# wangxuanx/Face-Diffusion-Model

Hardware: AMD Instinct MI355X
Metric: animated frames/sec (1000-step DDPM, VOCASET FDM) at 1/2/4/8 MI355X (higher is better)
Workload: dtype bf16; 1 GPU; cfg2: vocaset FDM, 4 clips/GPU x 200 latent frames, 1000-step DDPM, random-init weights, synthetic audio-encoder features, Philox noise; global_batch=4, latent_frames=200, diffusion_steps=1000, parallelism=clip-shard x1

## Files before the change

### face-diffusion-model_amd/csrc/fdm_hip.hip

```cpp
#include <hip/hip_runtime.h>

#include <algorithm>
#include <cstdarg>
#include <cstdio>
#include <cstring>
#include <functional>
#include <string>
#include <vector>

#include "../../include/fdm_hip.h"
#include "elementwise.hpp"
#include "window.hpp"
#include "kernels.hpp"

namespace fdm {
thread_local std::string g_err;
int fail(int code, const char* fmt, ...) {
  char buf[512];
  va_list ap;
  va_start(ap, fmt);
  vsnprintf(buf, sizeof(buf), fmt, ap);
  va_end(ap);
  g_err = buf;
  return code;
// ... 176 lines not shown
}

int fdm_op_layernorm(const fdm_ln_args* a, void* stream) {
  if (!a || !a->x || !a->gamma || !a->beta) return fail(FDM_ERR_ARG, "layernorm: null operand");
  if (a->d != 256 && a->d != 512 && a->d != 768 && a->d != 1024) return fail(FDM_ERR_SHAPE, "layernorm: d=%d unsupported (256, 512, 768, 1024)", a->d);
  if (a->M <= 0) return fail(FDM_ERR_SHAPE, "layernorm: M must be positive");
  if (!a->y_f32 && !a->y_t) return fail(FDM_ERR_ARG, "layernorm: no output");
  if (a->dtype < FDM_F32 || a->dtype > FDM_F16) return fail(FDM_ERR_ARG, "layernorm: bad dtype %d", a->dtype);
  if (a->y_t && a->dtype == FDM_F16X3 && (a->y_t_lo_off <= 0 || a->y_t_lo_off % 4)) return fail(FDM_ERR_ARG, "layernorm: split y_t needs y_t_lo_off");
  if (a->add_mat_group < 0 || a->add_mat_wrap < 0 ||
      (a->add_mat_group > 0 && (a->add_mat_L <= 0 || a->add_mat_group % a->add_mat_L || (a->add_mat_wrap > 0 && a->add_mat_wrap % a->add_mat_group))))
    return fail(FDM_ERR_SHAPE, "layernorm: shared add_mat needs add_mat_L | add_mat_group | add_mat_wrap (got %d, %d, %d)", a->add_mat_L, a->add_mat_group, a->add_mat_wrap);
  if (a->x_planes < 0 || a->x_planes > 4 || (a->x_planes > 1 && (a->x_plane_stride < (long long)a->M * a->d || a->x_plane_stride % 4)))
    return fail(FDM_ERR_ARG, "layernorm: x_planes %d (0..4) needs x_plane_stride >= M * d, a multiple of 4", a->x_planes);
  fdm_ln_args c = *a;
  return submit([c](hipStream_t s) {
    switch (c.dtype) {
      case FDM_BF16: return fdm::ln_launch_t<fdm::bf16>(c, s);
      case FDM_F16X3: return fdm::ln_launch_t<fdm::f16x3_t>(c, s);
      case FDM_F16: return fdm::ln_launch_t<fdm::f16>(c, s);
      default: return fdm::ln_launch_t<float>(c, s);
    }
  }, stream, "layernorm");
}

int fdm_op_sched_step(const fdm_sched_args* a, void* stream) {
  if (!a || !a->x0 || !a->x_out) return fail(FDM_ERR_ARG, "sched: null operand");
  if (a->n <= 0 || a->n % 4) return fail(FDM_ERR_SHAPE, "sched: n=%lld must be a positive multiple of 4", a->n);
  if (a->mode == 0 && (!a->x || !a->c1 || !a->c2 || !a->sigma)) return fail(FDM_ERR_ARG, "sched: DDPM tables missing");
  if (a->mode == 1 && (!a->x || !a->sra || !a->srm1 || !a->sqrt_an || !a->c_n)) return fail(FDM_ERR_ARG, "sched: DDIM tables missing");
  if (a->mode < 0 || a->mode > 2) return fail(FDM_ERR_ARG, "sched: bad mode %d", a->mode);
  if (a->mode == 0 && !a->noise && (a->n_per_clip <= 0 || a->n_per_clip % 4)) return fail(FDM_ERR_SHAPE, "sched: n_per_clip must be a positive multiple of 4");
  if (a->x_out_t && (a->out_dtype < FDM_F32 || a->out_dtype > FDM_F16)) return fail(FDM_ERR_ARG, "sched: bad out_dtype %d", a->out_dtype);
  if (a->x_out_t && a->out_dtype == FDM_F16X3 && (a->x_out_t_lo_off <= 0 || a->x_out_t_lo_off % 4)) return fail(FDM_ERR_ARG, "sched: split x_out_t needs x_out_t_lo_off");
  fdm_sched_args c = *a;
  return submit([c](hipStream_t s) { return fdm::sched_launch(c, s); }, stream, "sched");
}

}

int fdm::window_sched_op(const fdm_sched_args& a, const fdm::WinArgs& w, void* stream) {
  if (!a.x || !w.off || !w.ent || !w.xw || (!w.init && (!a.x0 || !a.x_out))) return fail(FDM_ERR_ARG, "window_sched: null operand");
  if (a.n <= 0 || a.n % 4 || w.d % 4 || w.L_total < 1 || w.W < 1 || w.n_win < 1 || a.n % ((long long)w.L_total * w.d))
    return fail(FDM_ERR_SHAPE, "window_sched: n=%lld is not a whole number of long clips of %d x %d", a.n, w.L_total, w.d);
  fdm_sched_args c = a;
  fdm::WinArgs ww = w;
// ... 279 lines not shown
```

### face-diffusion-model_amd/csrc/gemm_bf16.hip

```cpp
#include "gemm.hpp"
#include "kernels.hpp"
namespace fdm { hipError_t gemm_launch_bf16(const fdm_gemm_args& a, hipStream_t s) { return gemm_dispatch<bf16>(a, s); } }
namespace fdm {
int gemm_heuristic_tile_of(const fdm_gemm_args& a) {
  if (a.ksplit > 1) return gemm_ksplit_heuristic_tile(a);
  if (a.sched_fuse) {
    const bool pp = a.dtype != FDM_F16X3 && gemm_tile_override() == 0 && !a.ln_stat_in && a.N % 128 == 0 && gemm_sched_fuse_heuristic_pp(a, a.dtype == FDM_F32 ? 4 : 2);
    return pp ? FDM_TILE_256x128_PP : FDM_TILE_64x64;
  }
  const int want = gemm_tile_override();
  if (want > 0) return want;
  return gemm_heuristic_tile(a, a.dtype == FDM_F32 ? 4 : 2, a.dtype == FDM_F16X3);
}
}
```

### face-diffusion-model_amd/csrc/gemm_f16.hip

```cpp
#include "gemm.hpp"
#include "kernels.hpp"
namespace fdm { hipError_t gemm_launch_f16(const fdm_gemm_args& a, hipStream_t s) { return gemm_dispatch<f16>(a, s); } }
```

### face-diffusion-model_amd/csrc/kernels.hpp

```cpp
#pragma once
#include <hip/hip_runtime.h>
#include "../../include/fdm_hip.h"

namespace fdm {
int fail(int code, const char* fmt, ...);
hipError_t gemm_launch_f32(const fdm_gemm_args& a, hipStream_t s);
hipError_t gemm_launch_bf16(const fdm_gemm_args& a, hipStream_t s);
hipError_t gemm_launch_f16x3(const fdm_gemm_args& a, hipStream_t s);
hipError_t gemm_launch_f16(const fdm_gemm_args& a, hipStream_t s);
int gemm_heuristic_tile_of(const fdm_gemm_args& a);
hipError_t attn_launch_f32(const fdm_attn_args& a, hipStream_t s);
hipError_t attn_launch_bf16(const fdm_attn_args& a, hipStream_t s);
hipError_t attn_launch_f16x3(const fdm_attn_args& a, hipStream_t s);
hipError_t attn_launch_f16(const fdm_attn_args& a, hipStream_t s);
hipError_t pack_kv_launch_f32(const void* K, long long ldk, const void* V, long long ldv, void* Kp, void* Vp, int B, int H, int L, int Lpad, int hd, hipStream_t s);
hipError_t pack_kv_launch_bf16(const void* K, long long ldk, const void* V, long long ldv, void* Kp, void* Vp, int B, int H, int L, int Lpad, int hd, hipStream_t s);

struct WinEnt { int w; int start; float wt; int pad; };
struct WinArgs {
  const int* off; const WinEnt* ent;
  float* xw;
  int L_total;
  int n_win;
  int W;
  int d;
  int init;
};
int window_sched_op(const fdm_sched_args& p, const WinArgs& w, void* stream);

inline hipError_t gemm_launch(const fdm_gemm_args& a, hipStream_t s) {
  switch (a.dtype) {
    case FDM_BF16: return gemm_launch_bf16(a, s);
// ... 10 lines not shown
```

### face-diffusion-model_amd/csrc/plan.hip

```cpp
#include <hip/hip_runtime.h>

#include <algorithm>
#include <cmath>
#include <cstdint>
#include <cstdio>
#include <cstdlib>
#include <cstring>
#include <fstream>
#include <map>
#include <set>
#include <string>
#include <vector>

#include <unistd.h>

#include "../../include/fdm_hip.h"
#include "common.hpp"
#include "kernels.hpp"

namespace {
using fdm::fail;

#define HIPCK(x) do { hipError_t e_ = (x); if (e_ != hipSuccess) return fail(FDM_ERR_HIP, "%s: %s", #x, hipGetErrorString(e_)); } while (0)
#define FCK(x) do { int r_ = (x); if (r_ != FDM_OK) return r_; } while (0)
// ... 214 lines not shown
  void *q = nullptr, *kp = nullptr, *vp = nullptr;
  long long q_lo = 0, kv_lo = 0;
  size_t kv_bytes = 0;
  float *AF = nullptr, *t1 = nullptr, *sty = nullptr, *em = nullptr, *emu = nullptr, *zeros = nullptr, *E0 = nullptr;
  std::vector<float*> C1;
  int* step = nullptr;
  unsigned long long* seedbuf = nullptr;
  int* tseq = nullptr; int tseq_cap = 0;
  std::map<int, std::pair<int, float*>> ddim;
  std::map<int, std::vector<int>> ddim_t;
  std::map<std::string, fdm_prog*> progs;
  std::vector<std::string> prog_order;
  std::vector<std::string> pinned;
  std::map<std::string, int> tiles;
  std::map<std::string, std::map<std::string, int>> tile_cache;
  std::map<std::string, long long> steps_seen;
  std::map<std::string, std::vector<fdm_gemm_args>>* tune_rec = nullptr;
  int tune_enabled = 1;
  int tune_failed = 0;
  std::set<std::string> tune_failed_shapes;
  int want_fuse_ln3 = 0;
  int ksplit_out = 1, ksplit_ffn2 = 1;
  int x1_planes = 0;
  int lockstep = 0;
  int tune_lazy = 0;
  long long last_graph_launches = 0, launches_per_step = 0;
  int win_n = 0, win_len = 0, win_total = 0, win_overlap = 0, win_B = 0;
  float* xlong = nullptr; size_t xlong_cap = 0;
  int* win_off = nullptr; size_t win_off_cap = 0;
  fdm::WinEnt* win_ent = nullptr; size_t win_ent_cap = 0;
  float* win_stage = nullptr; size_t win_stage_cap = 0;
};

namespace {

size_t esize(int dtype) { return dtype == FDM_F32 ? 4 : 2; }
bool is_split(int dtype) { return dtype == FDM_F16X3; }

int dalloc(fdm_plan* P, void** out, size_t bytes, bool ws, bool zero = true) {
  void* p = nullptr;
  HIPCK(hipMalloc(&p, bytes ? bytes : 16));
  if (zero) HIPCK(hipMemset(p, 0, bytes ? bytes : 16));
  (ws ? P->ws_allocs : (P->in_commit ? P->commit_allocs : P->allocs)).push_back(p);
  *out = p;
  return FDM_OK;
}
// ... 37 lines not shown
  *out = w->p;
  return FDM_OK;
}

fdm_gemm_args gemm_f32(const float* A, const float* W, int M, int N, int K) {
  fdm_gemm_args a;
  memset(&a, 0, sizeof(a));
  a.A = A; a.lda = K; a.W = W; a.ldw = K; a.M = M; a.N = N; a.K = K; a.batch = 1; a.dtype = FDM_F32;
  a.ldr = N; a.ldo_f32 = N; a.ldo_t = N; a.ln_eps = 1e-5f;
  return a;
}
fdm_gemm_args gemm_op(const fdm_plan* P, const Mat& A, const Mat& W, int M, int N, int K) {
  fdm_gemm_args a = gemm_f32((const float*)A.p, (const float*)W.p, M, N, K);
  a.dtype = P->dtype; a.a_lo_off = A.lo; a.w_lo_off = W.lo;
  return a;
}
void set_out_t(fdm_gemm_args& a, const Mat& o) { a.out_t = o.p; a.out_t_lo_off = o.lo; }

int to_operand(fdm_plan* P, const float* src, long long n, Mat* out, void* stream) {
  if (P->dtype == FDM_F32) { out->p = (void*)src; out->lo = 0; return FDM_OK; }
  out->lo = is_split(P->dtype) ? n : 0;
  FCK(dalloc(P, &out->p, (size_t)n * 2 * (is_split(P->dtype) ? 2 : 1), false, false));
  return fdm_op_cast(src, out->p, n, P->dtype, stream);
}

int plan_gemm(fdm_plan* P, const char* label, fdm_gemm_args a, void* stream) {
  if (P->tune_rec) (*P->tune_rec)[label].push_back(a);
  auto it = P->tiles.find(label);
  a.tile = (it == P->tiles.end() ? 0 : it->second) | (P->lockstep ? FDM_TILE_LOCKSTEP : 0);
  return fdm_op_gemm(&a, stream);
}

std::string lname(int l, const char* suffix) {
  char b[96];
  snprintf(b, sizeof(b), "transformer_decoder.layers.%d.%s", l, suffix);
  return b;
}

int commit_impl(fdm_plan* P, void* stream) {
  const fdm_model_desc& m = P->m;
  const int d = m.d;
  hipStream_t s = (hipStream_t)stream;
  FCK(drop_programs(P, stream));
  const float* p = nullptr;
  FCK(need(P, "audio_extract.0.weight", (long long)d * m.audio_in, &p));
  FCK(need(P, "audio_extract.0.bias", d, &p));
// ... 225 lines not shown
    at.scale = 1.0f / std::sqrt((float)P->hd); at.causal = 1; at.slopes = P->slopes; at.period = m.period;
    if (split) { at.q_lo_off = P->q_lo; at.kv_lo_off = P->kv_lo; at.o_lo_off = P->ctx.lo; }
    FCK(fdm_op_attention(&at, stream));
    FCK(need(P, lname(l, "self_attn.out_proj.bias"), d, &b));
    g = gemm_op(P, P->ctx, P->wt[lname(l, "self_attn.out_proj.weight")], R, d, d);
    g.bias = b; g.out_f32 = P->x1;
    if (!f) {
      g.resid = P->h;
      if (P->ksplit_out > 1) { g.ksplit = P->ksplit_out; g.ksplit_stride = (long long)R * d; }
      FCK(plan_gemm(P, "out", g, stream));
    } else {
      g.resid = P->x2; g.ln_stat_in = P->stats; g.ln_nparts = np; g.ln_dim = d; g.ln_eps = eps; g.rln_gamma = f->gamma; g.rln_beta = f->beta;
      FCK(plan_gemm(P, "out_ln", g, stream));
    }
    fdm_ln_args ln;
    memset(&ln, 0, sizeof(ln));
    ln.x = P->x1; ln.M = R; ln.d = d; ln.add_mat = P->C1[l]; ln.add_tab = P->TT[l]; ln.tab_step = tcur; ln.eps = eps;
    if (P->S > 1) { ln.add_mat_L = L; ln.add_mat_group = P->S * L; ln.add_mat_wrap = M; }
    if (!f && P->ksplit_out > 1) { ln.x_planes = P->ksplit_out; ln.x_plane_stride = (long long)R * d; }
    FCK(need(P, lname(l, "norm1.weight"), d, &ln.gamma)); FCK(need(P, lname(l, "norm1.bias"), d, &ln.beta));
    FCK(need(P, lname(l, "norm2.weight"), d, &ln.gamma2)); FCK(need(P, lname(l, "norm2.bias"), d, &ln.beta2));
    ln.y_f32 = P->h2; ln.dtype = P->dtype;
    if (both) { ln.y_t = P->h2t.p; ln.y_t_lo_off = P->h2t.lo; }
    FCK(fdm_op_layernorm(&ln, stream));
    FCK(need(P, lname(l, "linear1.bias"), m.ffn, &b));
    g = gemm_op(P, P->h2t, P->wt[lname(l, "linear1.weight")], R, m.ffn, d);
    g.bias = b; g.act = FDM_ACT_RELU; set_out_t(g, P->u);
    FCK(plan_gemm(P, "ffn1", g, stream));
    FCK(need(P, lname(l, "linear2.bias"), d, &b));
    g = gemm_op(P, P->u, P->wt[lname(l, "linear2.weight")], R, d, m.ffn);
    g.bias = b; g.resid = P->h2;
    if (fuse) {
      g.out_f32 = P->x2; set_out_t(g, P->x2t); g.stat_out = P->stats;
      FCK(plan_gemm(P, "ffn2_stat", g, stream));
    } else {
      g.out_f32 = P->x1;
      if (P->ksplit_ffn2 > 1) { g.ksplit = P->ksplit_ffn2; g.ksplit_stride = (long long)R * d; }
      FCK(plan_gemm(P, "ffn2", g, stream));
      memset(&ln, 0, sizeof(ln));
      ln.x = P->x1; ln.M = R; ln.d = d; ln.eps = eps; ln.y_f32 = P->h; ln.dtype = P->dtype;
      if (P->ksplit_ffn2 > 1) { ln.x_planes = P->ksplit_ffn2; ln.x_plane_stride = (long long)R * d; }
      FCK(need(P, lname(l, "norm3.weight"), d, &ln.gamma)); FCK(need(P, lname(l, "norm3.bias"), d, &ln.beta));
      if (both) { ln.y_t = P->ht.p; ln.y_t_lo_off = P->ht.lo; }
      FCK(fdm_op_layernorm(&ln, stream));
    }
  }
  fdm_gemm_args g;
  if (fuse) {
    const Fold& f = P->fold[-1];
    g = gemm_op(P, P->x2t, f.w, R, d, d);
    g.bias = f.bias; g.ln_stat_in = P->stats; g.ln_nparts = np; g.ln_dim = d; g.ln_eps = eps; g.ln_colsum = f.colsum;
// ... 3 lines not shown
    g.bias = b;
  }
  if (sched) {
    g.resid = P->x; g.out_f32 = P->x;
    if (both) set_out_t(g, P->xt);
    g.sched_fuse = 1; g.sched = *sched;
  } else {
    g.out_f32 = P->x0;
  }
  return plan_gemm(P, fuse ? "dec_ln" : "dec", g, stream);
}

struct ProgSpec {
  int kind;
  const float* noise = nullptr; float cfg_scale = 0.f;
  const float* san = nullptr; const float* cn = nullptr;
  int reps = 1;
};

std::string tiles_sig(const fdm_plan* P) {
  std::string s;
  for (auto& kv : P->tiles)
    if (kv.second) s += kv.first + "=" + std::to_string(kv.second) + ",";
  s += "ks" + std::to_string(P->ksplit_out) + std::to_string(P->ksplit_ffn2) + (P->lockstep ? "L" : "");
  return s;
}

fdm::WinArgs win_args(const fdm_plan* P, int init) {
  fdm::WinArgs w;
  w.off = P->win_off; w.ent = P->win_ent; w.xw = P->x;
  w.L_total = P->win_total; w.n_win = P->win_n; w.W = P->win_len; w.d = P->m.d; w.init = init;
  return w;
}

int get_program(fdm_plan* P, const ProgSpec& sp, void* stream, fdm_prog** out) {
  char key[512];
  snprintf(key, sizeof(key), "%s#%s|%d|%p|%a|%p|%d", shape_key(P).c_str(), tiles_sig(P).c_str(), sp.kind, (const void*)sp.noise, (double)sp.cfg_scale,
           (const void*)sp.san, sp.reps);
  if (P->win_n) {
    const size_t kl = strlen(key);
    snprintf(key + kl, sizeof(key) - kl, "|win%d,%d,%d,%d,%d", P->win_B, P->win_total, P->win_n, P->win_len, P->win_overlap);
  }
  auto it = P->progs.find(key);
  if (it != P->progs.end()) {
    auto pos = std::find(P->prog_order.begin(), P->prog_order.end(), std::string(key));
    if (pos != P->prog_order.end()) { P->prog_order.erase(pos); P->prog_order.push_back(key); }
    P->pinned.push_back(key);
// ... 324 lines not shown
  if (any) {
    float t_h = 0.f, t_t = 0.f;
    FCK(chain_time({}, &t_h));
    FCK(chain_time(tuned, &t_t));
    for (auto& kv : runner_up) {
      std::map<std::string, int> trial = tuned;
      trial[kv.first] = kv.second;
      float t_a = 0.f;
      FCK(chain_time(trial, &t_a));
      if (t_a < 0.997f * t_t) { tuned = trial; t_t = t_a; }
    }
    if (t_t < 0.99f * t_h) {
      float t_h2 = 0.f;
      FCK(chain_time({}, &t_h2));
      t_h = std::min(t_h, t_h2);
    }
    if (t_t < 0.99f * t_h) keep = tuned;
    if (getenv("FDM_TUNE_VERBOSE")) {
      std::string desc;
      for (auto& kv : tuned) desc += kv.first + "=" + std::to_string(kv.second) + ",";
      fprintf(stderr, "[fdm tune] rows=%d candidates: %s chain %.3f -> %.3f ms: %s\n", P->R, desc.c_str(), t_h / 4, t_t / 4, keep.empty() ? "rejected" : "kept");
    }
  }
  P->tiles = keep;
  apply_tile_override(P->tiles);
  P->tile_cache[key] = P->tiles;
  return FDM_OK;
}

}

extern "C" {

int fdm_plan_create(const fdm_model_desc* desc, int B, int L, int cfg, int dtype, fdm_plan** out) {
  if (!desc || !out) return fail(FDM_ERR_ARG, "plan_create: null argument");
  if (dtype < FDM_F32 || dtype > FDM_F16) return fail(FDM_ERR_ARG, "plan_create: bad dtype %d", dtype);
  const fdm_model_desc& m = *desc;
  if (m.d <= 0 || m.n_head <= 0 || m.d % m.n_head || m.n_layers <= 0 || m.ffn <= 0 || m.G * m.c != m.d || m.pair <= 0 || m.max_len <= 0)
    return fail(FDM_ERR_SHAPE, "plan_create: inconsistent model geometry (d %d, heads %d, G*c %d)", m.d, m.n_head, m.G * m.c);
  const int hd = m.d / m.n_head;
  if (hd != 64 && hd != 128 && hd != 256) return fail(FDM_ERR_SHAPE, "plan_create: head_dim %d unsupported (64, 128, 256)", hd);
  if (m.d != 256 && m.d != 512 && m.d != 768 && m.d != 1024) return fail(FDM_ERR_SHAPE, "plan_create: feature_dim %d unsupported (256, 512, 768, 1024)", m.d);
  if (B < 1 || L < 1 || L > m.max_len) return fail(FDM_ERR_SHAPE, "plan_create: B=%d, L=%d outside [1, .] x [1, %d] (models/fdm_vocaset.py:44)", B, L, m.max_len);
  if (!fdm_device_ok()) return fail(FDM_ERR_STATE, "plan_create: no gfx950 device visible (there is no CPU fallback)");
  fdm_plan* P = new (std::nothrow) fdm_plan();
  if (!P) return fail(FDM_ERR_STATE, "plan_create: out of memory");
// ... 291 lines not shown
int fdm_sample_graph(fdm_plan* P, const fdm_sample_args* a, void* stream) {
  FCK(check_ready(P));
  if (P->win_n) return fail(FDM_ERR_STATE, "sample_graph: the plan was prepared for windowed sampling (fdm_sample_windows)");
  return sample_impl(P, a, stream);
}

int fdm_sample_windows(fdm_plan* P, const fdm_sample_args* a, void* stream) {
  FCK(check_ready(P));
  if (!P->win_n) return fail(FDM_ERR_STATE, "sample_windows: call fdm_audio_prepare_windows first");
  return sample_impl(P, a, stream);
}

int fdm_plan_tune(fdm_plan* P, void* stream) {
  FCK(check_ready(P));
  return tune_tiles(P, 1, stream);
}

int fdm_plan_get(fdm_plan* P, const char* key, long long* out) {
  if (!P || !key || !out) return fail(FDM_ERR_ARG, "plan_get: null argument");
  const std::string k(key);
  if (k == "launches_per_step") *out = P->launches_per_step;
  else if (k == "graph_launches") *out = P->last_graph_launches;
  else if (k == "fuse_ln3") *out = P->fuse_ln3;
  else if (k == "rows") *out = P->R;
  else if (k == "ksplit.out") *out = P->ksplit_out;
  else if (k == "ksplit.ffn2") *out = P->ksplit_ffn2;
  else if (k == "tuned") *out = P->tile_cache.count(shape_key(P)) ? 1 : 0;
  else if (k == "needs_tune") { const std::string sk = shape_key(P); *out = (!P->tile_cache.count(sk) && P->tune_enabled && P->steps_seen.count(sk) && P->steps_seen[sk] >= 2000 && !P->tune_failed_shapes.count(sk)) ? 1 : 0; }
  else if (k == "tune_failed") *out = P->tune_failed;
  else if (k == "windows") *out = P->win_n;
  else if (k == "window_len") *out = P->win_n ? P->win_len : P->L;
  else if (k == "L_total") *out = P->win_n ? P->win_total : P->L;
  else if (k.rfind("tile.", 0) == 0) { auto it = P->tiles.find(k.substr(5)); *out = it == P->tiles.end() ? 0 : it->second; }
  else return fail(FDM_ERR_ARG, "plan_get: unknown key '%s'", key);
  return FDM_OK;
}

int fdm_plan_set(fdm_plan* P, const char* key, long long value) {
  if (!P || !key) return fail(FDM_ERR_ARG, "plan_set: null argument");
  const std::string k(key);
  if (k == "tune") { P->tune_enabled = value != 0; return FDM_OK; }
  if (k == "tune_lazy") { P->tune_lazy = value != 0; return FDM_OK; }
  if (k == "fuse_ln3") {
    if ((value != 0) != (P->want_fuse_ln3 != 0)) { P->want_fuse_ln3 = value != 0; P->committed = false; P->prepared = false; return drop_programs(P, nullptr); }
    return FDM_OK;
  }
  if (k == "ksplit.out" || k == "ksplit.ffn2") {
    const int kt = (k == "ksplit.out" ? P->m.d : P->m.ffn) / (P->dtype == FDM_F32 ? 32 : 64);
    if (value < 1 || value > 4 || kt % value) return fail(FDM_ERR_ARG, "plan_set: %s = %lld must be 1..4 and divide the %d k-tiles", key, value, kt);
    int& cur = k == "ksplit.out" ? P->ksplit_out : P->ksplit_ffn2;
    if (cur == (int)value) return FDM_OK;
    cur = (int)value;
    P->tile_cache.clear(); P->tiles.erase(k == "ksplit.out" ? "out" : "ffn2");
    FCK(drop_programs(P, nullptr));
    if (P->capB > 0 && (int)value > P->x1_planes) {
      P->x1_planes = (int)value;
      FCK(dalloc_t(P, &P->x1, (size_t)P->capB * P->capL * P->capRep * P->m.d * P->x1_planes, true));
    }
    return FDM_OK;
  }
  if (k == "lockstep") { P->lockstep = value != 0; P->tile_cache.clear(); P->tiles.clear(); return drop_programs(P, nullptr); }
  if (k == "untune") {
    P->tile_cache.clear(); P->steps_seen.clear(); P->tiles.clear(); P->tune_failed_shapes.clear();
    return drop_programs(P, nullptr);
  }
  if (k.rfind("tile.", 0) == 0) {
    if (value < 0 || value > FDM_TILE_MAX) return fail(FDM_ERR_ARG, "plan_set: unknown tile %lld", value);
    P->tiles[k.substr(5)] = (int)value;
    P->tile_cache[shape_key(P)] = P->tiles;
    return drop_programs(P, nullptr);
  }
  return fail(FDM_ERR_ARG, "plan_set: unknown key '%s'", key);
}

}
```

### face-diffusion-model_amd/fdm_amd/_lib.py

```python
import ctypes as C
import os

_HERE = os.path.dirname(os.path.abspath(__file__))
LIB_PATH = os.environ.get("FDM_LIB_PATH") or os.path.join(_HERE, "libfdm_hip.so")

F32, BF16, F16X3, F16 = 0, 1, 2, 3
DTYPE_NAMES = {"f32": F32, "bf16": BF16, "f16x3": F16X3, "f16": F16}
ACT_NONE, ACT_RELU, ACT_MISH, ACT_GELU_ERF, ACT_GELU_TANH, ACT_LEAKY02 = range(6)

vp, ll, ci, cf = C.c_void_p, C.c_longlong, C.c_int, C.c_float


class SchedArgs(C.Structure):
    _fields_ = [("x0", vp), ("x0u", vp), ("cfg_scale", cf), ("x", vp), ("x_out", vp),
                ("n", ll), ("n_per_clip", ll), ("tseq", vp), ("step", vp), ("advance", ci),
                ("c1", vp), ("c2", vp), ("sigma", vp), ("sra", vp), ("srm1", vp),
                ("sqrt_an", vp), ("c_n", vp), ("noise", vp), ("noise_stride", ll), ("x_out_t", vp), ("out_dtype", ci), ("arrive", vp),
                ("seed", C.c_ulonglong), ("clip0", ci),
                ("mode", ci), ("x_out_t_lo_off", ll), ("seed_dev", vp)]


class GemmArgs(C.Structure):
    _fields_ = [("A", vp), ("lda", ll), ("a_batch_stride", ll),
                ("W", vp), ("ldw", ll), ("w_batch_stride", ll),
# ... 35 lines not shown
                ("scale", cf), ("causal", ci), ("slopes", vp), ("period", ci), ("o_split", ci), ("o_lo_off", ll), ("q_lo_off", ll), ("kv_lo_off", ll)]


class LnArgs(C.Structure):
    _fields_ = [("x", vp), ("M", ci), ("d", ci), ("add_mat", vp), ("add_tab", vp),
                ("tab_index", vp), ("tab_step", vp), ("gamma", vp), ("beta", vp), ("eps", cf),
                ("act", ci), ("y_f32", vp), ("y_t", vp), ("dtype", ci), ("gamma2", vp), ("beta2", vp), ("y_t_lo_off", ll),
                ("add_mat_L", ci), ("add_mat_group", ci), ("add_mat_wrap", ci), ("x_planes", ci), ("x_plane_stride", ll)]


STRUCTS = {"fdm_sched_args": SchedArgs, "fdm_gemm_args": GemmArgs, "fdm_attn_args": AttnArgs, "fdm_ln_args": LnArgs,
           "fdm_model_desc": ModelDesc, "fdm_sample_args": SampleArgs, "fdm_vq_desc": VqDesc}

SYMBOLS = {
    "fdm_last_error": (C.c_char_p, []),
    "fdm_version": (ci, []),
    "fdm_abi_struct_size": (ci, [C.c_char_p]),
    "fdm_device_ok": (ci, []),
    "fdm_op_gemm": (ci, [C.POINTER(GemmArgs), vp]),
    "fdm_gemm_heuristic_tile": (ci, [C.POINTER(GemmArgs)]),
    "fdm_op_attention": (ci, [C.POINTER(AttnArgs), vp]),
    "fdm_op_pack_kv": (ci, [vp, ll, vp, ll, vp, vp, ci, ci, ci, ci, ci, ci, vp]),
    "fdm_op_layernorm": (ci, [C.POINTER(LnArgs), vp]),
    "fdm_op_sched_step": (ci, [C.POINTER(SchedArgs), vp]),
    "fdm_op_cast": (ci, [vp, vp, ll, ci, vp]),
    "fdm_op_vertex_err": (ci, [vp, vp, vp, ci, ci, ci, vp, vp, vp, vp]),
    "fdm_op_motion_std": (ci, [vp, vp, vp, ci, ci, ci, vp, vp, vp]),
    "fdm_op_linear_interp": (ci, [vp, vp, ci, ci, ci, ci, vp]),
    "fdm_op_bias_act": (ci, [vp, vp, vp, ll, ci, ci, vp]),
    "fdm_op_add_rows": (ci, [vp, ci, ci, vp, ci, ci, vp, ci, ci, vp, ll, ci, vp]),
    "fdm_op_small_linear": (ci, [vp, vp, vp, vp, ci, ci, ci, ci, vp]),
    "fdm_op_pad_rows": (ci, [vp, vp, ci, ci, ci, ci, ci, ci, vp]),
    "fdm_op_group_pad": (ci, [vp, vp, ci, ci, ci, ci, ci, ci, vp]),
    "fdm_op_conv0": (ci, [vp, vp, vp, vp, ci, ci, ci, vp]),
    "fdm_op_conv0_ln_gelu": (ci, [vp, vp, vp, vp, vp, vp, ll, ci, ci, ci, cf, ci, vp]),
    "fdm_op_leaky_instnorm": (ci, [vp, vp, vp, ci, ci, ci, cf, ci, vp]),
    "fdm_op_adain": (ci, [vp, vp, vp, ci, ci, ci, cf, vp]),
    "fdm_op_mean_diff": (ci, [vp, vp, vp, vp, ll, ci, vp]),
    "fdm_op_time_groupnorm": (ci, [vp, vp, vp, vp, vp, ll, ci, ci, ci, cf, ci, ci, vp, ll, vp]),
    "fdm_op_vq_quant": (ci, [vp, vp, vp, ci, ci, ci, ci, vp, vp, vp]),
    "fdm_op_vq_stats": (ci, [vp, vp, vp, vp, ci, ci, ci, ci, cf, vp, vp, vp, vp, vp]),
    "fdm_prog_create": (ci, [C.POINTER(vp)]),
    "fdm_prog_destroy": (ci, [vp]),
    "fdm_prog_begin": (ci, [vp]),
    "fdm_prog_end": (ci, [vp]),
    "fdm_prog_run": (ci, [vp, vp]),
# ... 73 lines not shown
```

### face-diffusion-model_amd/fdm_amd/ops.py

```python
import ctypes as C

import torch

from . import _lib
from ._lib import (ACT_GELU_ERF, ACT_GELU_TANH, ACT_LEAKY02, ACT_MISH, ACT_NONE, ACT_RELU, BF16, F16, F16X3, F32,
                   AttnArgs, GemmArgs, LnArgs, SchedArgs, check, lib)


class Split:

    def __init__(self, planes, code, row0=0, col0=0):
        self.planes, self.code, self.row0, self.col0 = planes, code, row0, col0
        self.lo_off = planes[0].numel()

    @classmethod
    def empty(cls, rows, cols, code, device):
        return cls(torch.zeros(2, rows, cols, device=device, dtype=tdtype(code)), code)

    def __getitem__(self, sl):
        if not isinstance(sl, slice) or sl.stop is not None or sl.step is not None:
            raise _lib.FdmError("Split operands support [r0:] row offsets only")
        return Split(self.planes, self.code, self.row0 + (sl.start or 0), self.col0)

    @property
# ... 104 lines not shown
def attention(Q, Kp, Vp, O, *, B, H, L, hd, ldq, ldo, Lpad, scale, causal=False, slopes=None, period=1):
    a = AttnArgs()
    a.Q, a.ldq, a.Kp, a.Vp, a.Lpad = _p(Q), ldq, _p(Kp), _p(Vp), Lpad
    a.O, a.ldo, a.B, a.H, a.L, a.hd, a.dtype = _p(O), ldo, B, H, L, hd, code_of(Q)
    if isinstance(Q, Split):
        a.q_lo_off, a.kv_lo_off, a.o_lo_off = Q.lo_off, Kp.lo_off, O.lo_off
    elif isinstance(O, Split):
        a.o_split, a.o_lo_off = O.code, O.lo_off
    a.scale, a.causal, a.slopes, a.period = scale, int(causal), _p(slopes), period
    check(lib().fdm_op_attention(C.byref(a), stream()))


def layernorm(x, gamma, beta, M, d, *, add_mat=None, add_tab=None, tab_index=None, tab_step=None, eps=1e-5,
              act=ACT_NONE, y_f32=None, y_t=None, dtype=F32, gamma2=None, beta2=None, x_planes=0, x_plane_stride=0):
    a = LnArgs()
    a.x, a.M, a.d, a.add_mat, a.add_tab = _p(x), M, d, _p(add_mat), _p(add_tab)
    a.tab_index, a.tab_step, a.gamma, a.beta, a.eps = _p(tab_index), _p(tab_step), _p(gamma), _p(beta), eps
    a.act, a.y_f32, a.y_t, a.dtype = act, _p(y_f32), _p(y_t), dtype
    a.gamma2, a.beta2, a.y_t_lo_off = _p(gamma2), _p(beta2), _lo(y_t)
    a.x_planes, a.x_plane_stride = x_planes, x_plane_stride
    check(lib().fdm_op_layernorm(C.byref(a), stream()))


def sched_args(mode, x0, x, x_out, n, *, x0u=None, cfg_scale=0.0, n_per_clip=0, tseq=None, step=None, advance=0,
               c1=None, c2=None, sigma=None, sra=None, srm1=None, sqrt_an=None, c_n=None, noise=None, noise_stride=0,
               seed=0, clip0=0, x_out_t=None, arrive=None):
    a = SchedArgs()
    a.x0, a.x0u, a.cfg_scale, a.x, a.x_out = _p(x0), _p(x0u), cfg_scale, _p(x), _p(x_out)
    a.n, a.n_per_clip, a.tseq, a.step, a.advance = n, n_per_clip, _p(tseq), _p(step), advance
    a.c1, a.c2, a.sigma, a.sra, a.srm1 = _p(c1), _p(c2), _p(sigma), _p(sra), _p(srm1)
    a.sqrt_an, a.c_n, a.noise, a.noise_stride = _p(sqrt_an), _p(c_n), _p(noise), noise_stride
    a.seed, a.clip0, a.mode = seed, clip0, mode
    a.x_out_t, a.out_dtype, a.arrive = _p(x_out_t), (code_of(x_out_t) if x_out_t is not None else 0), _p(arrive)
    a.x_out_t_lo_off = _lo(x_out_t)
    return a


def sched_step(mode, x0, x, x_out, n, **kw):
    a = sched_args(mode, x0, x, x_out, n, **kw)
    check(lib().fdm_op_sched_step(C.byref(a), stream()))


def cast(src, dst):
    check(lib().fdm_op_cast(_p(src), _p(dst), src.numel(), code_of(dst), stream()))


# ... 117 lines not shown
```

### include/fdm_hip.h

```cpp
#ifndef FDM_HIP_H
#define FDM_HIP_H

#ifdef __cplusplus
extern "C" {
#endif

#define FDM_F32 0
#define FDM_BF16 1
#define FDM_F16X3 2
#define FDM_F16 3

#define FDM_ACT_NONE 0
#define FDM_ACT_RELU 1
#define FDM_ACT_MISH 2
#define FDM_ACT_GELU_ERF 3
#define FDM_ACT_GELU_TANH 4
#define FDM_ACT_LEAKY02 5

#define FDM_OK 0
#define FDM_ERR_ARG (-1)
#define FDM_ERR_SHAPE (-2)
#define FDM_ERR_HIP (-3)
#define FDM_ERR_STATE (-4)

// ... 81 lines not shown
  int period;
  int o_split; long long o_lo_off;
  long long q_lo_off, kv_lo_off;
} fdm_attn_args;
int fdm_op_attention(const fdm_attn_args* a, void* stream);
int fdm_op_pack_kv(const void* K, long long ldk, const void* V, long long ldv, void* Kp, void* Vp,
                   int B, int H, int L, int Lpad, int hd, int dtype, void* stream);

typedef struct fdm_ln_args {
  const float* x; int M, d;
  const float* add_mat;
  const float* add_tab;
  const int* tab_index; const int* tab_step;
  const float* gamma; const float* beta; float eps;
  int act;
  float* y_f32; void* y_t; int dtype;
  const float* gamma2; const float* beta2;
  long long y_t_lo_off;
  int add_mat_L, add_mat_group, add_mat_wrap;
  int x_planes; long long x_plane_stride;
} fdm_ln_args;
int fdm_op_layernorm(const fdm_ln_args* a, void* stream);


int fdm_op_cast(const float* src, void* dst, long long n, int dtype, void* stream);
int fdm_op_bias_act(const float* in, const float* vec, float* out, long long rows, int d, int act, void* stream);
int fdm_op_add_rows(const float* a, int a_div, int a_mod, const float* b, int b_div, int b_mod,
                    const float* c, int c_div, int c_mod, float* out, long long M, int d, void* stream);
int fdm_op_small_linear(const float* x, const float* W, const float* bias, float* out, int B, int K, int d,
                        int act, void* stream);
int fdm_op_pad_rows(const void* in, void* out, int B, int L, int d, int pad, int dtype, int zero, void* stream);
int fdm_op_conv0(const float* wav, const float* w, const float* bias, float* out, int B, int n, int T0, void* stream);
int fdm_op_conv0_ln_gelu(const float* wav, const float* w, const float* bias, const float* gamma, const float* beta, void* out,
                         long long out_lo_off, int B, int n, int T0, float eps, int dtype, void* stream);
int fdm_op_leaky_instnorm(const float* x, float* y_f32, void* y_t, int B, int L, int d, float eps, int dtype, void* stream);
int fdm_op_time_groupnorm(const float* x, const float* gamma, const float* beta, float* y_f32, void* y_t, long long y_t_lo_off, int B, int T, int C,
                          float eps, int act, int dtype, void* scratch, long long scratch_bytes, void* stream);
int fdm_op_mean_diff(const float* a, const float* b, float* partial, float* out, long long n, int l1, void* stream);
int fdm_op_vertex_err(const float* gt, const float* pred, const int* region, int R, int F, int V,
                      float* frame_max, double* frame_sum, double* out, void* stream);
int fdm_op_motion_std(const float* verts, const float* tmpl, const int* region, int R, int F, int V,
                      double* partial, double* out, void* stream);
int fdm_op_linear_interp(const float* x, float* y, int B, int Tin, int Tout, int C, void* stream);
int fdm_op_adain(const float* content, const float* style, float* out, int NC, int Lc, int Ls, float eps, void* stream);
int fdm_op_group_pad(const void* in, void* out, int B, int T, int d, int groups, int pad, int dtype, void* stream);

// ... 88 lines not shown
```

Before: 1890 frames/s.

## Fuse double LayerNorm into FFN1 GEMM prologue with LDS-resident activation panel

Adds a GEMM kernel that computes the fused two-stage LayerNorm (norm, add embeddings, norm2) for a 64-row tile directly into an LDS panel, then runs the FFN1 GEMM against a warp-specialised W ring loaded with global_load_lds. This removes the separate LayerNorm launch and the round trip of the normalised bf16 activations through global memory. Each column block recomputes the LayerNorm for its rows, which is redundant work across N/128 blocks. It uses a large LDS footprint that limits occupancy. The path is autotuned and only kept if the chain timing improves by at least 1%.

```diff
diff --git a/face-diffusion-model_amd/csrc/fdm_hip.hip b/face-diffusion-model_amd/csrc/fdm_hip.hip
--- a/face-diffusion-model_amd/csrc/fdm_hip.hip
+++ b/face-diffusion-model_amd/csrc/fdm_hip.hip
@@ -222,6 +222,35 @@
       default: return fdm::ln_launch_t<float>(c, s);
     }
   }, stream, "layernorm");
+}
+
+int fdm_op_gemm_ln(const fdm_gemm_args* g, const fdm_ln_args* ln, void* stream) {
+  if (!g || !ln || !g->W || !ln->x) return fail(FDM_ERR_ARG, "gemm_ln: null operand");
+  if (g->dtype != FDM_BF16 && g->dtype != FDM_F16) return fail(FDM_ERR_ARG, "gemm_ln: dtype %d (the one-plane 16-bit kinds FDM_BF16 / FDM_F16 only: a split or fp32 panel does not fit the LDS)", g->dtype);
+  if (ln->dtype != g->dtype) return fail(FDM_ERR_ARG, "gemm_ln: the LayerNorm and the GEMM must name the same operand kind");
+  if (g->M <= 0 || ln->M != g->M) return fail(FDM_ERR_SHAPE, "gemm_ln: rows must be positive and equal (%d, %d)", g->M, ln->M);
+  if (ln->d != 1024 || g->K != 1024) return fail(FDM_ERR_SHAPE, "gemm_ln: d = K = 1024 only (d %d, K %d)", ln->d, g->K);
+  if (g->N <= 0 || g->N % 128) return fail(FDM_ERR_SHAPE, "gemm_ln: N=%d must be a positive multiple of 128", g->N);
+  if (!ln->gamma || !ln->beta || !ln->gamma2 || !ln->beta2 || !ln->add_mat || !ln->add_tab || !ln->y_f32)
+    return fail(FDM_ERR_ARG, "gemm_ln: needs the fused form (gamma, beta, gamma2, beta2, add_mat, add_tab) and y_f32");
+  if (ln->act != FDM_ACT_NONE || ln->x_planes > 1) return fail(FDM_ERR_ARG, "gemm_ln: no LayerNorm activation, one x plane");
+  if (ln->add_mat_group < 0 || ln->add_mat_wrap < 0 ||
+      (ln->add_mat_group > 0 && (ln->add_mat_L <= 0 || ln->add_mat_group % ln->add_mat_L || (ln->add_mat_wrap > 0 && ln->add_mat_wrap % ln->add_mat_group))))
+    return fail(FDM_ERR_SHAPE, "gemm_ln: shared add_mat needs add_mat_L | add_mat_group | add_mat_wrap (got %d, %d, %d)", ln->add_mat_L, ln->add_mat_group, ln->add_mat_wrap);
+  if (!aligned16(ln->x) || !aligned16(ln->add_mat) || !aligned16(ln->add_tab) || !aligned16(ln->y_f32) || !aligned16(ln->gamma) || !aligned16(ln->beta) ||
+      !aligned16(ln->gamma2) || !aligned16(ln->beta2))
+    return fail(FDM_ERR_ARG, "gemm_ln: LayerNorm operands must be 16-byte aligned");
+  if (g->ldw % 8 || g->ldw < g->K || g->ldw > 0x7fffffffLL || !aligned16(g->W)) return fail(FDM_ERR_ARG, "gemm_ln: W needs 16-byte aligned rows of at least K elements");
+  if (g->batch > 1 || g->batch2 >= 1 || g->ksplit > 1 || g->out_batch_stride || g->out_kp || g->out_vp || g->stat_out || g->ln_stat_in || g->ln_colsum || g->rln_gamma ||
+      g->sched_fuse || g->resid_row_mod || g->incr_counter || gemm_act_heavy_host(g->act))
+    return fail(FDM_ERR_ARG, "gemm_ln: needs a plain GEMM (one batch, no K slices, packed K/V, LayerNorm folds, fused scheduler, step counter or Mish/GELU)");
+  if (!g->out_f32 && !g->out_t) return fail(FDM_ERR_ARG, "gemm_ln: no output");
+  if ((g->out_f32 && (g->ldo_f32 % 4 || !aligned16(g->out_f32))) || (g->out_t && (g->ldo_t % 4 || ((uintptr_t)g->out_t & 7))) || (g->resid && (g->ldr % 4 || !aligned16(g->resid))) ||
+      (g->bias && !aligned16(g->bias)))
+    return fail(FDM_ERR_ARG, "gemm_ln: outputs, residual and bias need vectorisable rows");
+  fdm_gemm_args c = *g;
+  fdm_ln_args l = *ln;
+  return submit([c, l](hipStream_t s) { return c.dtype == FDM_BF16 ? fdm::gemm_lnp_launch_bf16(c, l, s) : fdm::gemm_lnp_launch_f16(c, l, s); }, stream, "gemm_ln");
 }
 
 int fdm_op_sched_step(const fdm_sched_args* a, void* stream) {
diff --git a/face-diffusion-model_amd/csrc/gemm_bf16.hip b/face-diffusion-model_amd/csrc/gemm_bf16.hip
--- a/face-diffusion-model_amd/csrc/gemm_bf16.hip
+++ b/face-diffusion-model_amd/csrc/gemm_bf16.hip
@@ -1,6 +1,8 @@
 #include "gemm.hpp"
+#include "gemm_lnp.hpp"
 #include "kernels.hpp"
 namespace fdm { hipError_t gemm_launch_bf16(const fdm_gemm_args& a, hipStream_t s) { return gemm_dispatch<bf16>(a, s); } }
+namespace fdm { hipError_t gemm_lnp_launch_bf16(const fdm_gemm_args& a, const fdm_ln_args& q, hipStream_t s) { return gemm_lnp_launch_t<bf16>(a, q, s); } }
 namespace fdm {
 int gemm_heuristic_tile_of(const fdm_gemm_args& a) {
   if (a.ksplit > 1) return gemm_ksplit_heuristic_tile(a);
diff --git a/face-diffusion-model_amd/csrc/gemm_f16.hip b/face-diffusion-model_amd/csrc/gemm_f16.hip
--- a/face-diffusion-model_amd/csrc/gemm_f16.hip
+++ b/face-diffusion-model_amd/csrc/gemm_f16.hip
@@ -1,3 +1,5 @@
 #include "gemm.hpp"
+#include "gemm_lnp.hpp"
 #include "kernels.hpp"
 namespace fdm { hipError_t gemm_launch_f16(const fdm_gemm_args& a, hipStream_t s) { return gemm_dispatch<f16>(a, s); } }
+namespace fdm { hipError_t gemm_lnp_launch_f16(const fdm_gemm_args& a, const fdm_ln_args& q, hipStream_t s) { return gemm_lnp_launch_t<f16>(a, q, s); } }
diff --git a/face-diffusion-model_amd/csrc/gemm_lnp.hpp b/face-diffusion-model_amd/csrc/gemm_lnp.hpp
--- /dev/null
+++ b/face-diffusion-model_amd/csrc/gemm_lnp.hpp
@@ -0,0 +1,194 @@
+#pragma once
+#include "gemm.hpp"
+
+namespace fdm {
+
+template <typename T>
+__global__ __launch_bounds__(768) void gemm_lnp_kernel(const void* pW, const float* p_x, const float* p_add_mat, const float* p_add_tab, const int* p_tab_step,
+                                                       int pM, int pN, int p_ldw, const fdm_gemm_args p, const fdm_ln_args q) {
+  using E = typename Opnd<T>::E;
+  static_assert(Opnd<T>::NP == 1 && sizeof(E) == 2, "one-plane 16-bit operand kinds only");
+  constexpr int BM = 64, BN = 128, WM = 2, WN = 4, NW = WM * WN, LW = 4, NST = 4, D = 1024;
+  constexpr int ROWB = 64, RPI = 1024 / ROWB, MI = BM / WM / 16, NI = BN / WN / 16;
+  constexpr int W_IPW = BN / RPI / LW;
+  constexpr int STAGE = BN * ROWB, PANEL = BM * D * 2, PROW = D * 2;
+  constexpr int NK = D / 32;
+  extern __shared__ __attribute__((aligned(16))) char smem[];
+  char* panel = smem;
+  char* ring = smem + PANEL;
+
+  const int tid = threadIdx.x, lane = tid & 63;
+  const int wave_id = __builtin_amdgcn_readfirstlane(tid >> 6);
+  const bool loader = wave_id >= NW;
+  const int lw = loader ? wave_id - NW : 0;
+  const int wm = wave_id / WN, wn = wave_id % WN;
+  const int g = lane >> 4, r16 = lane & 15;
+  const int m0 = blockIdx.y * BM, n0 = blockIdx.x * BN;
+  const int M = pM, N = pN;
+  auto swz = [](int row) { return (0x78 >> (2 * ((row >> 2) & 3))) & 3; };
+
+  const int lrow = lane / 4, slot = lane % 4;
+  auto issue = [&](int kt) {
+    char* sb = ring + (kt % NST) * STAGE;
+#pragma unroll
+    for (int i = 0; i < W_IPW; ++i) {
+      const int row = RPI * (lw * W_IPW + i) + lrow;
+      const char* src = (const char*)((const E*)pW + (size_t)min(n0 + row, N - 1) * p_ldw) + ((slot ^ swz(row)) << 4);
+      __builtin_amdgcn_global_load_lds((gptr_t)(src + (size_t)kt * ROWB), (lptr_t)(sb + (lw * W_IPW + i) * 1024), 16, 0, 0);
+    }
+  };
+  if (loader) {
+#pragma unroll
+    for (int t = 0; t < NST - 1; ++t) issue(t);
+  }
+
+  {
+    f32x4 g1[4], b1[4], g2[4], b2[4], et[4];
+    const int c4 = 4 * lane;
+#pragma unroll
+    for (int w = 0; w < 4; ++w) {
+      g1[w] = *(const f32x4*)(q.gamma + 256 * w + c4); b1[w] = *(const f32x4*)(q.beta + 256 * w + c4);
+      g2[w] = *(const f32x4*)(q.gamma2 + 256 * w + c4); b2[w] = *(const f32x4*)(q.beta2 + 256 * w + c4);
+    }
+    {
+      const int k = p_tab_step ? *p_tab_step : 0;
+      const int idx = q.tab_index ? q.tab_index[k] : k;
+#pragma unroll
+      for (int w = 0; w < 4; ++w) et[w] = *(const f32x4*)(p_add_tab + (size_t)idx * D + 256 * w + c4);
+    }
+    const int nbx = gridDim.x;
+    const int cw = (((D + nbx - 1) / nbx) + 3) & ~3;
+    const int c_lo = blockIdx.x * cw, c_hi = min(c_lo + cw, D);
+    auto row_sum = [&](const float (&a)[4]) {
+      float s[4];
+#pragma unroll
+      for (int w = 0; w < 4; ++w) s[w] = wave_sum(a[w]);
+      float t = 0.f;
+#pragma unroll
+      for (int w = 0; w < 4; ++w) t += s[w];
+      return t;
+    };
+#pragma clang loop unroll(disable)
+    for (int r = wave_id; r < BM; r += NW + LW) {
+      const int row = m0 + r;
+      char* prow = panel + r * PROW + (lane & 1) * 8;
+      const int sw = r & 15, ch = lane >> 1;
+      if (row >= M) {
+#pragma unroll
+        for (int w = 0; w < 4; ++w) *(u32x2*)(prow + (((32 * w + ch) ^ sw) << 4)) = u32x2{0u, 0u};
+        continue;
+      }
+      int arow = row;
+      if (q.add_mat_group > 0) {
+        const int m = q.add_mat_wrap > 0 ? row % q.add_mat_wrap : row;
+        arow = (m / q.add_mat_group) * q.add_mat_L + m % q.add_mat_L;
+      }
+      const float* xr = p_x + (size_t)row * D + c4;
+      const float* er = p_add_mat + (size_t)arow * D + c4;
+      f32x4 v[4], e[4];
+      float a[4];
+#pragma unroll
+      for (int w = 0; w < 4; ++w) v[w] = *(const f32x4*)(xr + 256 * w);
+#pragma unroll
+      for (int w = 0; w < 4; ++w) e[w] = *(const f32x4*)(er + 256 * w);
+#pragma unroll
+      for (int w = 0; w < 4; ++w) a[w] = (v[w][0] + v[w][1]) + (v[w][2] + v[w][3]);
+      float mean = row_sum(a) * (1.f / D);
+#pragma unroll
+      for (int w = 0; w < 4; ++w) {
+        v[w] -= mean;
+        a[w] = (v[w][0] * v[w][0] + v[w][1] * v[w][1]) + (v[w][2] * v[w][2] + v[w][3] * v[w][3]);
+      }
+      float var = row_sum(a) * (1.f / D);
+      float rstd = 1.f / sqrtf(var + q.eps);
+#pragma unroll
+      for (int w = 0; w < 4; ++w) {
+        v[w] = v[w] * rstd * g1[w] + b1[w];
+        v[w] += e[w] + et[w];
+        a[w] = (v[w][0] + v[w][1]) + (v[w][2] + v[w][3]);
+      }
+      mean = row_sum(a) * (1.f / D);
+#pragma unroll
+      for (int w = 0; w < 4; ++w) {
+        v[w] -= mean;
+        a[w] = (v[w][0] * v[w][0] + v[w][1] * v[w][1]) + (v[w][2] * v[w][2] + v[w][3] * v[w][3]);
+      }
+      var = row_sum(a) * (1.f / D);
+      rstd = 1.f / sqrtf(var + q.eps);
+      float* yr = q.y_f32 + (size_t)row * D + c4;
+#pragma unroll
+      for (int w = 0; w < 4; ++w) {
+        const f32x4 y = v[w] * rstd * g2[w] + b2[w];
+        const int col = 256 * w + c4;
+        if (col >= c_lo && col < c_hi) st16(yr + 256 * w, y);
+        typedef __attribute__((ext_vector_type(4))) E e4;
+        e4 o;
+#pragma unroll
+        for (int j = 0; j < 4; ++j) o[j] = (E)(std::is_same<E, f16>::value ? clamp_f16(y[j]) : y[j]);
+        *(u32x2*)(prow + (((32 * w + ch) ^ sw) << 4)) = __builtin_bit_cast(u32x2, o);
+      }
+    }
+  }
+
+  if (loader) {
+    asm volatile("s_waitcnt vmcnt(0) lgkmcnt(0)" ::: "memory");
+    for (int kt = 0; kt < NK; ++kt) {
+      if (kt + NST - 2 < NK) wait_vmcnt<(NST - 2) * W_IPW>();
+      else wait_vmcnt<0>();
+      __builtin_amdgcn_s_barrier();
+      if (kt + NST - 1 < NK) issue(kt + NST - 1);
+    }
+    return;
+  }
+
+  EpiPre<MI, NI> epre;
+  gemm_epi_preload<T, BM, BN, WM, WN, false>(p, m0, n0, 0, wm, wn, g, r16, false, epre);
+  f32x4 acc[MI][NI];
+#pragma unroll
+  for (int mi = 0; mi < MI; ++mi)
+#pragma unroll
+    for (int ni = 0; ni < NI; ++ni) acc[mi][ni] = f32x4{0.f, 0.f, 0.f, 0.f};
+  int a_off[MI], w_off[NI];
+#pragma unroll
+  for (int mi = 0; mi < MI; ++mi) {
+    const int row = wm * (BM / WM) + mi * 16 + r16;
+    a_off[mi] = row * PROW;
+  }
+#pragma unroll
+  for (int ni = 0; ni < NI; ++ni) {
+    const int row = wn * (BN / WN) + ni * 16 + r16;
+    w_off[ni] = row * ROWB + ((g ^ swz(row)) << 4);
+  }
+  asm volatile("s_waitcnt lgkmcnt(0)" ::: "memory");
+  for (int kt = 0; kt < NK; ++kt) {
+    __builtin_amdgcn_s_barrier();
+    const char* base = ring + (kt % NST) * STAGE;
+    u32x4 af[MI], wf[NI];
+#pragma unroll
+    for (int mi = 0; mi < MI; ++mi) af[mi] = *(const u32x4*)(panel + a_off[mi] + (((4 * kt + g) ^ r16) << 4));
+#pragma unroll
+    for (int ni = 0; ni < NI; ++ni) wf[ni] = *(const u32x4*)(base + w_off[ni]);
+#pragma unroll
+    for (int mi = 0; mi < MI; ++mi)
+#pragma unroll
+      for (int ni = 0; ni < NI; ++ni) Mma<T>::run(acc[mi][ni], wf[ni], af[mi]);
+  }
+  wait_vmcnt<0>();
+  gemm_epilogue<T, BM, BN, WM, WN, false, false, GEMM_LEAN>(p, acc, epre, m0, n0, 0, wm, wn, g, r16, nullptr, nullptr);
+}
+
+template <typename T>
+static hipError_t gemm_lnp_launch_t(const fdm_gemm_args& a, const fdm_ln_args& q, hipStream_t s) {
+  if (a.N % 128 || a.K != 1024 || q.d != 1024 || !gemm_all_tiles_lean<T, 64, 128>(a)) return hipErrorInvalidValue;
+  constexpr int lds = 64 * 1024 * 2 + 4 * 128 * 64;
+  static_assert(lds <= 160 * 1024, "panel + ring do not fit the CU's LDS");
+  static bool once = [] {
+    return hipFuncSetAttribute((const void*)gemm_lnp_kernel<T>, hipFuncAttributeMaxDynamicSharedMemorySize, lds) == hipSuccess;
+  }();
+  (void)once;
+  dim3 grid(a.N / 128, (a.M + 63) / 64, 1);
+  hipLaunchKernelGGL((gemm_lnp_kernel<T>), grid, dim3(768), lds, s, a.W, q.x, q.add_mat, q.add_tab, q.tab_step, a.M, a.N, (int)a.ldw, a, q);
+  return hipGetLastError();
+}
+
+}
diff --git a/face-diffusion-model_amd/csrc/kernels.hpp b/face-diffusion-model_amd/csrc/kernels.hpp
--- a/face-diffusion-model_amd/csrc/kernels.hpp
+++ b/face-diffusion-model_amd/csrc/kernels.hpp
@@ -8,6 +8,8 @@
 hipError_t gemm_launch_bf16(const fdm_gemm_args& a, hipStream_t s);
 hipError_t gemm_launch_f16x3(const fdm_gemm_args& a, hipStream_t s);
 hipError_t gemm_launch_f16(const fdm_gemm_args& a, hipStream_t s);
+hipError_t gemm_lnp_launch_bf16(const fdm_gemm_args& a, const fdm_ln_args& q, hipStream_t s);
+hipError_t gemm_lnp_launch_f16(const fdm_gemm_args& a, const fdm_ln_args& q, hipStream_t s);
 int gemm_heuristic_tile_of(const fdm_gemm_args& a);
 hipError_t attn_launch_f32(const fdm_attn_args& a, hipStream_t s);
 hipError_t attn_launch_bf16(const fdm_attn_args& a, hipStream_t s);
diff --git a/face-diffusion-model_amd/csrc/plan.hip b/face-diffusion-model_amd/csrc/plan.hip
--- a/face-diffusion-model_amd/csrc/plan.hip
+++ b/face-diffusion-model_amd/csrc/plan.hip
@@ -260,6 +260,7 @@
   int want_fuse_ln3 = 0;
   int ksplit_out = 1, ksplit_ffn2 = 1;
   int x1_planes = 0;
+  int ln_prologue = -1;
   int lockstep = 0;
   int tune_lazy = 0;
   long long last_graph_launches = 0, launches_per_step = 0;
@@ -343,6 +344,16 @@
   out->lo = is_split(P->dtype) ? n : 0;
   FCK(dalloc(P, &out->p, (size_t)n * 2 * (is_split(P->dtype) ? 2 : 1), false, false));
   return fdm_op_cast(src, out->p, n, P->dtype, stream);
+}
+
+bool ln_prologue_ok(const fdm_plan* P) {
+  return (P->dtype == FDM_BF16 || P->dtype == FDM_F16) && P->m.d == 1024 && P->m.ffn % 128 == 0 && P->ksplit_out <= 1 && !P->fuse_ln3 && !P->win_n;
+}
+bool ln_prologue_on(const fdm_plan* P) {
+  if (!ln_prologue_ok(P) || P->ln_prologue == 0) return false;
+  if (P->ln_prologue > 0) return true;
+  auto it = P->tiles.find("ffn1.lnp");
+  return it != P->tiles.end() && it->second == 1;
 }
 
 int plan_gemm(fdm_plan* P, const char* label, fdm_gemm_args a, void* stream) {
@@ -614,11 +625,17 @@
     FCK(need(P, lname(l, "norm2.weight"), d, &ln.gamma2)); FCK(need(P, lname(l, "norm2.bias"), d, &ln.beta2));
     ln.y_f32 = P->h2; ln.dtype = P->dtype;
     if (both) { ln.y_t = P->h2t.p; ln.y_t_lo_off = P->h2t.lo; }
-    FCK(fdm_op_layernorm(&ln, stream));
+    const bool lnp = ln_prologue_on(P);
+    if (!lnp) FCK(fdm_op_layernorm(&ln, stream));
     FCK(need(P, lname(l, "linear1.bias"), m.ffn, &b));
     g = gemm_op(P, P->h2t, P->wt[lname(l, "linear1.weight")], R, m.ffn, d);
     g.bias = b; g.act = FDM_ACT_RELU; set_out_t(g, P->u);
-    FCK(plan_gemm(P, "ffn1", g, stream));
+    if (lnp) {
+      if (P->tune_rec) (*P->tune_rec)["ffn1"].push_back(g);
+      FCK(fdm_op_gemm_ln(&g, &ln, stream));
+    } else {
+      FCK(plan_gemm(P, "ffn1", g, stream));
+    }
     FCK(need(P, lname(l, "linear2.bias"), d, &b));
     g = gemm_op(P, P->u, P->wt[lname(l, "linear2.weight")], R, d, m.ffn);
     g.bias = b; g.resid = P->h2;
@@ -668,7 +685,7 @@
   std::string s;
   for (auto& kv : P->tiles)
     if (kv.second) s += kv.first + "=" + std::to_string(kv.second) + ",";
-  s += "ks" + std::to_string(P->ksplit_out) + std::to_string(P->ksplit_ffn2) + (P->lockstep ? "L" : "");
+  s += "ks" + std::to_string(P->ksplit_out) + std::to_string(P->ksplit_ffn2) + (P->lockstep ? "L" : "") + (ln_prologue_on(P) ? "P" : "");
   return s;
 }
 
@@ -1039,6 +1056,16 @@
       fprintf(stderr, "[fdm tune] rows=%d candidates: %s chain %.3f -> %.3f ms: %s\n", P->R, desc.c_str(), t_h / 4, t_t / 4, keep.empty() ? "rejected" : "kept");
     }
   }
+  if (P->ln_prologue < 0 && ln_prologue_ok(P)) {
+    float t_off = 0.f, t_on = 0.f, t_off2 = 0.f;
+    std::map<std::string, int> trial = keep;
+    trial["ffn1.lnp"] = 1;
+    FCK(chain_time(keep, &t_off));
+    FCK(chain_time(trial, &t_on));
+    if (t_on < 0.99f * t_off) { FCK(chain_time(keep, &t_off2)); t_off = std::min(t_off, t_off2); }
+    if (getenv("FDM_TUNE_VERBOSE")) fprintf(stderr, "[fdm tune] rows=%d ln_prologue: chain %.3f -> %.3f ms: %s\n", P->R, t_off, t_on, t_on < 0.99f * t_off ? "kept" : "rejected");
+    if (t_on < 0.99f * t_off) keep = trial;
+  }
   P->tiles = keep;
   apply_tile_override(P->tiles);
   P->tile_cache[key] = P->tiles;
@@ -1376,6 +1403,8 @@
   if (k == "launches_per_step") *out = P->launches_per_step;
   else if (k == "graph_launches") *out = P->last_graph_launches;
   else if (k == "fuse_ln3") *out = P->fuse_ln3;
+  else if (k == "ln_prologue") *out = P->ln_prologue;
+  else if (k == "ln_prologue_on") *out = ln_prologue_on(P) ? 1 : 0;
   else if (k == "rows") *out = P->R;
   else if (k == "ksplit.out") *out = P->ksplit_out;
   else if (k == "ksplit.ffn2") *out = P->ksplit_ffn2;
@@ -1413,6 +1442,12 @@
     }
     return FDM_OK;
   }
+  if (k == "ln_prologue") {
+    if (value < -1 || value > 1) return fail(FDM_ERR_ARG, "plan_set: ln_prologue = %lld must be -1, 0 or 1", value);
+    if (P->ln_prologue == (int)value) return FDM_OK;
+    P->ln_prologue = (int)value;
+    return drop_programs(P, nullptr);
+  }
   if (k == "lockstep") { P->lockstep = value != 0; P->tile_cache.clear(); P->tiles.clear(); return drop_programs(P, nullptr); }
   if (k == "untune") {
     P->tile_cache.clear(); P->steps_seen.clear(); P->tiles.clear(); P->tune_failed_shapes.clear();
diff --git a/face-diffusion-model_amd/fdm_amd/_lib.py b/face-diffusion-model_amd/fdm_amd/_lib.py
--- a/face-diffusion-model_amd/fdm_amd/_lib.py
+++ b/face-diffusion-model_amd/fdm_amd/_lib.py
@@ -81,6 +81,7 @@
     "fdm_op_attention": (ci, [C.POINTER(AttnArgs), vp]),
     "fdm_op_pack_kv": (ci, [vp, ll, vp, ll, vp, vp, ci, ci, ci, ci, ci, ci, vp]),
     "fdm_op_layernorm": (ci, [C.POINTER(LnArgs), vp]),
+    "fdm_op_gemm_ln": (ci, [C.POINTER(GemmArgs), C.POINTER(LnArgs), vp]),
     "fdm_op_sched_step": (ci, [C.POINTER(SchedArgs), vp]),
     "fdm_op_cast": (ci, [vp, vp, ll, ci, vp]),
     "fdm_op_vertex_err": (ci, [vp, vp, vp, ci, ci, ci, vp, vp, vp, vp]),
diff --git a/face-diffusion-model_amd/fdm_amd/ops.py b/face-diffusion-model_amd/fdm_amd/ops.py
--- a/face-diffusion-model_amd/fdm_amd/ops.py
+++ b/face-diffusion-model_amd/fdm_amd/ops.py
@@ -150,6 +150,21 @@
     check(lib().fdm_op_layernorm(C.byref(a), stream()))
 
 
+def gemm_ln(x, gamma, beta, gamma2, beta2, add_mat, add_tab, W, M, N, *, tab_index=None, tab_step=None, eps=1e-5, y_f32,
+            add_mat_L=0, add_mat_group=0, add_mat_wrap=0, bias=None, act=ACT_NONE, resid=None, out_f32=None, out_t=None):
+    a = LnArgs()
+    a.x, a.M, a.d, a.add_mat, a.add_tab = _p(x), M, 1024, _p(add_mat), _p(add_tab)
+    a.tab_index, a.tab_step, a.gamma, a.beta, a.eps = _p(tab_index), _p(tab_step), _p(gamma), _p(beta), eps
+    a.act, a.y_f32, a.dtype = ACT_NONE, _p(y_f32), code_of(W)
+    a.gamma2, a.beta2 = _p(gamma2), _p(beta2)
+    a.add_mat_L, a.add_mat_group, a.add_mat_wrap = add_mat_L, add_mat_group, add_mat_wrap
+    g = GemmArgs()
+    g.W, g.ldw, g.M, g.N, g.K, g.batch, g.dtype = _p(W), 1024, M, N, 1024, 1, code_of(W)
+    g.bias, g.act, g.resid, g.ldr = _p(bias), act, _p(resid), N
+    g.out_f32, g.ldo_f32, g.out_t, g.ldo_t = _p(out_f32), N, _p(out_t), N
+    check(lib().fdm_op_gemm_ln(C.byref(g), C.byref(a), stream()))
+
+
 def sched_args(mode, x0, x, x_out, n, *, x0u=None, cfg_scale=0.0, n_per_clip=0, tseq=None, step=None, advance=0,
                c1=None, c2=None, sigma=None, sra=None, srm1=None, sqrt_an=None, c_n=None, noise=None, noise_stride=0,
                seed=0, clip0=0, x_out_t=None, arrive=None):
diff --git a/include/fdm_hip.h b/include/fdm_hip.h
--- a/include/fdm_hip.h
+++ b/include/fdm_hip.h
@@ -127,6 +127,8 @@
 } fdm_ln_args;
 int fdm_op_layernorm(const fdm_ln_args* a, void* stream);
 
+int fdm_op_gemm_ln(const fdm_gemm_args* g, const fdm_ln_args* ln, void* stream);
+
 
 int fdm_op_cast(const float* src, void* dst, long long n, int dtype, void* stream);
 int fdm_op_bias_act(const float* in, const float* vec, float* out, long long rows, int d, int act, void* stream);
```

Result: slower. 1843 frames/s (-2.5%).
